# jermp/sshash

Measured on AMD Instinct MI355X. Metric: k-mer Lookups/sec (batched random queries, bit-exact ids), higher is better.
Workload: dtype u64

## Files before the change

sshash_amd/_binding.py:

```python
from __future__ import annotations

import ctypes as C
import os
import sys
from dataclasses import dataclass
from typing import Callable, Iterable, Optional, Sequence, Union

import numpy as np

INVALID_U64 = 0xFFFFFFFFFFFFFFFF

_HERE = os.path.dirname(os.path.abspath(__file__))
_LIB_NAME = "libsshash_amd.so"


def library_path() -> str:
    return os.environ.get("SSHASH_AMD_LIBRARY") or os.path.join(_HERE, _LIB_NAME)


class SSHashError(RuntimeError):

    def __init__(self, status: int, message: str):
        super().__init__(f"[sshash status {status}] {message}")
        self.status = status
# ... 326 lines not shown
    def weighted(self) -> bool: return bool(self._info.weighted)

    def to_device(self, device: int = 0, table_shards: int = 1, table_shard_id: int = 0) -> "Dictionary":
        if table_shards > 1:
            _check(_load().sshash_to_device_table_shard(self._h, int(device), int(table_shards), int(table_shard_id)))
            return self
        _check(_load().sshash_to_device(self._h, int(device)))
        return self

    def device_bytes(self, device: int = 0) -> int:
        out = C.c_uint64()
        _check(_load().sshash_device_bytes(self._h, int(device), C.byref(out)))
        return int(out.value)

    def bucket_stats(self) -> dict:
        out = (C.c_uint64 * 64)()
        _check(_load().sshash_bucket_stats(self._h, C.byref(out)))
        v = [int(x) for x in out]
        return {"num_minimizers": v[0], "num_minimizer_positions": v[1], "num_buckets_larger_than_1_not_in_skew_index": v[2],
                "num_minimizer_positions_of_buckets_larger_than_1": v[3], "num_buckets_in_skew_index": v[4],
                "num_minimizer_positions_of_buckets_in_skew_index": v[5], "num_kmers_in_skew_index": v[6], "max_bucket_size": v[7],
                "num_kmers_in_skew_partition": v[8:8 + v[35]], "buckets_with_n_positions": v[16:32], "num_kmers": v[32],
                "num_strings": v[33], "num_bases": v[34], "max_string_length": v[36]}

    def device_stats(self, device: int = 0) -> dict:
        out = (C.c_uint64 * 16)()
        _check(_load().sshash_device_stats(self._h, int(device), C.byref(out)))
        reasons = {0: None, 1: "disabled", 2: "minimizer shard", 3: "more than 2^39 bases", 4: "too many items for one build pass",
                   5: "not enough free HBM"}
        return {"bytes": int(out[0]), "directory_sectors": int(out[1]), "directory_overflow_sectors": int(out[2]),
                "directory_keys": int(out[3]), "sk_slots": int(out[4]), "sk_keys": int(out[5]), "sk_inline_keys": int(out[6]),
                "sk_deferred_keys": int(out[7]), "sk_slots_used": int(out[8]), "sk_heavy_keys": int(out[9]),
                "sk_heavy_kmers": int(out[10]), "sk_absent_reason": reasons.get(int(out[11]), str(int(out[11]))),
                "sk_bytes": int(out[12]), "sk_key_length": int(out[13]), "sk_load_factor": round(int(out[8]) / int(out[4]), 4) if int(out[4]) else 0.0}

    def device_table_histogram(self, device: int = 0) -> dict:
        out = (C.c_uint64 * 32)()
        _check(_load().sshash_device_table_histogram(self._h, int(device), C.byref(out)))
        v = [int(x) for x in out]
        bins = ["1", "2", "3", "4", "5-8", "9-16", "17-64", "65-1024", ">1024"]
        return {"keys_by_occurrences": dict(zip(bins, v[0:9])), "super_kmers_by_occurrences_of_their_key": dict(zip(bins, v[9:18])),
                "super_kmers": v[18], "slots_asked_for": v[19]}

    def _as_batch(self, kmers: KmerBatch):
        if isinstance(kmers, (str, bytes)):
            kmers = [kmers]
        if isinstance(kmers, np.ndarray) and kmers.dtype == np.uint64:
            a = np.ascontiguousarray(kmers)
            w = self.words_per_kmer()
            if a.size % w:
                raise ValueError("packed k-mer array length is not a multiple of words_per_kmer")
            return False, a, a.size // w
        if isinstance(kmers, np.ndarray) and kmers.dtype == np.uint8:
            a = np.ascontiguousarray(kmers)
            if a.size % self.k():
                raise ValueError("ASCII k-mer buffer length is not a multiple of k")
            return True, a, a.size // self.k()
        a = encode_kmers(list(kmers), self.k())
        return True, np.ascontiguousarray(a), a.shape[0]

    def lookup(self, kmers: KmerBatch, check_reverse_complement: bool = True, full: bool = False,
               out: Optional[np.ndarray] = None) -> LookupResult:
        is_ascii, a, n = self._as_batch(kmers)
        if out is not None and (out.dtype != np.uint64 or out.size != n or not out.flags["C_CONTIGUOUS"]):
            raise ValueError("out must be a contiguous uint64 array with one entry per k-mer")
        res = LookupResult(kmer_id=out if out is not None else np.empty(n, dtype=np.uint64))
        r = _Results()
# ... 393 lines not shown
```

sshash_amd/csrc/engine.hip:

```cpp
#include <hip/hip_runtime.h>

#include <algorithm>
#include <atomic>
#include <cstdlib>
#include <cstring>
#include <mutex>
#include <exception>
#include <stdexcept>
#include <thread>

#include "engine.hpp"
#include "hooks.hpp"
#include "replica.hpp"
#include "sktable.hpp"

namespace sshash_amd {

static void check_single_launch(uint64_t lanes, char const* what) {
    if (lanes >= (uint64_t(1) << 32))
        throw error(error_kind::argument, std::string(what) + ": at most 2^32 - 1 lanes per call (split the batch)");
}


int visible_device_count() {
// ... 124 lines not shown
    std::shared_lock<std::shared_mutex> lock(m_replicas_mutex);
    for (auto const& r : m_replicas)
        if (r->device == device) return true;
    return false;
}

std::vector<int> engine::devices() const {
    std::vector<int> d;
    std::shared_lock<std::shared_mutex> lock(m_replicas_mutex);
    for (auto const& r : m_replicas) d.push_back(r->device);
    return d;
}

uint64_t engine::device_bytes(int device) const { return replica(device)->bytes; }

void engine::device_stats(int device, uint64_t out[16]) const {
    device_replica const* r = replica(device);
    out[0] = r->bytes;
    out[1] = r->view.directory.enabled ? r->view.directory.num_buckets : 0;
    out[2] = r->directory_overflowed;
    out[3] = r->directory_entries;
    out[4] = r->view.sk.enabled ? uint64_t(r->view.sk.num_buckets) * SK_BUCKET_SLOTS +
                                      uint64_t(r->view.sk.kmer_buckets) * (r->view.k > 31 ? SK_BUCKET_SLOTS : SK_KMER_ENTRIES_NARROW)
                                : 0;
    out[5] = r->sk_keys;
    out[6] = r->sk_keys - r->sk_heavy_keys;
    out[7] = r->sk_unplaced;
    out[8] = r->sk_slots_used;
    out[9] = r->sk_heavy_keys;
    out[10] = r->sk_heavy_kmers;
    out[11] = r->view.sk.enabled ? 0 : r->sk_absent_reason;
    out[12] = r->sk_bytes;
    out[13] = r->view.sk.m;
    out[14] = out[15] = 0;
}

void engine::device_table_histogram(int device, uint64_t out[32]) const {
    device_replica const* r = replica(device);
    for (int i = 0; i < 32; ++i) out[i] = i < 20 && r->view.sk.enabled ? r->sk_histogram[i] : 0;
}

device_replica const* engine::replica(int device) const {
    std::shared_lock<std::shared_mutex> lock(m_replicas_mutex);
    for (auto const& r : m_replicas)
        if (r->device == device) return r.get();
    throw error(error_kind::no_device, "dictionary is not resident on device " + std::to_string(device) +
                             " (call sshash_to_device first)");
}

char const* isa_guard_state() {
#if defined(SSHASH_ISA_GUARDED)
    return "guarded";
#else
    return "plain";
#endif
}

void engine::to_device(int device, uint32_t table_shards, uint32_t table_shard_id) {
#if !defined(SSHASH_ISA_GUARDED)
    {
        static std::once_flag once;
        std::call_once(once, [] {
            fprintf(stderr, "[sshash_amd] WARNING: this library was NOT built through tools/isa_guard.py (make -C sshash_amd/csrc): on gfx950 a "
                                "kernel that keeps a 64-bit shift amount in the last VGPR of its allocation computes wrongly some of the time "
                                "(HISTORY.md); tests/test_isa_guard.py names the kernels of a build that are exposed\n");
        });
    }
// ... 32 lines not shown
        std::vector<granule> g = make_granules(idx, nt);
        if (idx.k <= 31) {
            std::vector<atom32> a = make_atoms(g, nt);
            std::vector<granule>().swap(g);
            v.granules = rep->put(a);
        } else {
            v.granules = rep->put(g);
        }
    }
    v.endpoints = rep->put(idx.endpoints);
    v.minimizers = rep->put_mphf(idx.minimizers_mphf);
    v.cw_width = idx.control_codewords.width;
    v.off_width = idx.mid_load_buckets.width;
    v.begin_buckets_of_size = rep->put(idx.begin_buckets_of_size);
    v.mid_load = rep->put(idx.mid_load_buckets.words);
    v.heavy_load = rep->put(idx.heavy_load_buckets.words);
    v.heavy_size = idx.heavy_load_buckets.size;
    v.codewords = nullptr;
    v.cw_packed = 0;
    v.directory.buckets = nullptr;
    v.directory.num_buckets = 0;
    v.directory.enabled = 0;
    rep->bytes_still_to_come = 8 * sizeof(skew_part_dev);
    for (uint32_t p = 0; p < 8; ++p) {
        if (p < idx.skew_num_partitions && idx.skew_mphfs[p].num_keys) {
            mphf_host const& f = idx.skew_mphfs[p];
            rep->bytes_still_to_come += f.parts.size() * sizeof(f.parts[0]) + (f.pilots.size() + f.free_slots.size() + idx.skew_positions[p].words.size()) * 8;
        } else {
            rep->bytes_still_to_come += 64;
        }
    }
    if (idx.weighted()) rep->bytes_still_to_come += (idx.weight_starts.size() + idx.weight_values.size()) * 8;
    build_sk_table(*rep, idx, table_shards, table_shard_id);
    const char* dir_env = std::getenv("SSHASH_AMD_DIRECTORY");
    const bool lean = v.sk.enabled && !(dir_env && dir_env[0] == '1');
    if (lean) {
        v.codewords = rep->put(idx.control_codewords.words);
        v.cw_packed = 1;
    } else {
        const uint64_t n = idx.control_codewords.size;
        device_buffers tmp;
        uint64_t* packed = tmp.alloc<uint64_t>(idx.control_codewords.words.size());
        HIP_CHECK(hipMemcpy(packed, idx.control_codewords.words.data(), idx.control_codewords.words.size() * sizeof(uint64_t), hipMemcpyHostToDevice));
        uint64_t* wide = tmp.alloc<uint64_t>(std::max<uint64_t>(n, 1));
        tmp.keep(wide, *rep);
        rep->bytes += std::max<uint64_t>(n, 1) * sizeof(uint64_t);
        if (n) {
            check_single_launch(n, "upload (one lane per minimizer)");
            hipLaunchKernelGGL(widen_codewords_kernel, dim3(uint32_t((n + 255) / 256)), dim3(256), 0, 0, v, packed, n, wide);
            HIP_CHECK(hipGetLastError());
            HIP_CHECK(hipDeviceSynchronize());
        }
        v.codewords = wide;
    }
    if (!lean) {
        const bool want = !(dir_env && dir_env[0] == '0');
        const uint64_t n = idx.control_codewords.size;
        const uint64_t nb = uint64_t(double(n) / DIR_LOAD) + 1;
        if (want && n && nb < (uint64_t(1) << 32) && v.cw_width <= DIR_CODE_BITS) {
            device_buffers tmp;
            uint64_t* buckets = tmp.alloc<uint64_t>(nb * 4);
            uint32_t* claimed = tmp.alloc<uint32_t>(nb);
            unsigned long long* stats = tmp.alloc<unsigned long long>(2);
            HIP_CHECK(hipMemset(buckets, 0, nb * 32));
            HIP_CHECK(hipMemset(claimed, 0, nb * 4));
            HIP_CHECK(hipMemset(stats, 0, 16));
// ... 76 lines not shown
    }
}

constexpr uint32_t DEFER_SHARDS = 2048;
constexpr uint32_t DEFER_BLOCKS_PER_SHARD = 4;

struct pass_queues {
    uint32_t* defer_counts;
    uint32_t* resume_counts;
    uint32_t* defer_index;
    uint32_t* resume_index;
    uint64_t* resume_kmers;
    uint64_t* resume_meta;
    uint32_t defer_capacity;
    uint32_t resume_capacity;
    uint32_t flag_misses;
};
constexpr uint32_t DEFER_FLAG_ONLY = 1u << 31;

template <int W, bool ASCII>
__device__ __forceinline__ kmer_w<W> load_query(const void* __restrict__ queries, uint64_t i, uint32_t k) {
    kmer_w<W> x;
    if constexpr (ASCII) {
        x = kmer_from_ascii<W>(static_cast<const char*>(queries) + i * k, k);
    } else {
        const uint64_t* q = static_cast<const uint64_t*>(queries) + i * W;
        for (int j = 0; j < W; ++j) x.w[j] = __builtin_nontemporal_load(q + j);
        x = kmer_take_chars<W>(x, k);
    }
    return x;
}

template <int W, bool CANON, int MODE, bool ASCII, bool SK>
__global__ void __launch_bounds__(256, (W == 2 && SK) ? 8 : 1)
fast_lookup_kernel(const dict_view d, const void* __restrict__ queries, const uint64_t n, const bool check_rc,
                   const result_view out, uint8_t* __restrict__ member, const pass_queues q,
                   const uint8_t* __restrict__ lane_valid ) {
    constexpr uint32_t TILE_WORDS = ASCII ? 64 * (W == 1 ? 31 : 63) + 24 : 0;
    constexpr uint32_t STAGE_WORDS = SK ? 256 * 16 : 0;
    __shared__ uint4 lds[(TILE_WORDS > STAGE_WORDS ? TILE_WORDS : STAGE_WORDS) / 4 + 1];
    const uint64_t i = uint64_t(blockIdx.x) * blockDim.x + threadIdx.x;
    const bool active = i < n && (!lane_valid || (lane_valid[i] & 1));
    kmer_w<W> x = kmer_zero<W>();
    if constexpr (ASCII) {
        uint32_t* tile = reinterpret_cast<uint32_t*>(lds);
        const uint64_t first = uint64_t(blockIdx.x) * blockDim.x;
        const uint32_t count = uint32_t(n - first < blockDim.x ? n - first : blockDim.x);
        const uint32_t bytes = count * d.k;
        const char* src = static_cast<const char*>(queries) + first * d.k;
        if ((reinterpret_cast<uintptr_t>(src) & 15) == 0) {
            for (uint32_t c = threadIdx.x; c * 16 < bytes; c += blockDim.x) {
                if (c * 16 + 16 <= bytes) {
                    reinterpret_cast<uint4*>(tile)[c] = sk_load_piece(src + 16 * c);
                } else {
                    for (uint32_t b = c * 16; b < bytes; ++b) reinterpret_cast<char*>(tile)[b] = src[b];
                }
            }
        } else {
            for (uint32_t b = threadIdx.x; b < bytes; b += blockDim.x) reinterpret_cast<char*>(tile)[b] = src[b];
        }
        __syncthreads();
        if (active) {
            const uint32_t start = threadIdx.x * d.k, w0 = start >> 2, sh = start & 3;
            uint32_t acc[2 * W];
#pragma unroll
            for (int t = 0; t < 2 * W; ++t) {
                acc[t] = 0;
                if (16u * uint32_t(t) < d.k) {
                    uint32_t prev = tile[w0 + 4 * t];
#pragma unroll
                    for (int j = 0; j < 4; ++j) {
                        const uint32_t next = tile[w0 + 4 * t + j + 1];
                        const uint32_t four = __builtin_amdgcn_alignbyte(next, prev, sh);
                        prev = next;
                        const uint32_t c = (((four >> 1) & 0x03030303u) * 0x01041040u) >> 24;
                        acc[t] |= c << (8 * j);
                    }
                }
            }
            x.w[0] = uint64_t(acc[0]) | (uint64_t(acc[1]) << 32);
            if constexpr (W == 2) x.w[1] = uint64_t(acc[2]) | (uint64_t(acc[3]) << 32);
            x = kmer_take_chars<W>(x, d.k);
        }
        if constexpr (SK) __syncthreads();
    } else {
        if (active) x = load_query<W, false>(queries, i, d.k);
    }
    fast_t r;
    const uint32_t shard = blockIdx.x & (DEFER_SHARDS - 1);
    if constexpr (SK) {
        if constexpr (W == 1)
            r = sk_lookup_in_wave<W>(d, x, active, CANON || check_rc, (!CANON && check_rc) ? int8_t(-1) : int8_t(1), lds + (threadIdx.x >> 6) * (64 * 4));
        else
            r = sk_first_pass_wave<W>(d, x, active, CANON || check_rc, (!CANON && check_rc) ? int8_t(-1) : int8_t(1),
                                      lds + (threadIdx.x >> 6) * (64 * 4));
        bool resume = active && r.outcome == FAST_CONTINUE;
        const uint32_t place = wave_queue_place(resume, q.resume_counts + shard);
        if (resume) {
            if (place < q.resume_capacity) {
                const uint64_t at = uint64_t(shard) * q.resume_capacity + place;
                q.resume_index[at] = uint32_t(i) | uint32_t(r.kmer_offset);
                for (int j = 0; j < W; ++j) q.resume_kmers[at * W + j] = x.w[j];
            } else {
                r.outcome = FAST_DEFER;
            }
        }
        if (!active) return;
    } else {
        bool by_pairs = false;
        if constexpr (W == 1 && !CANON) by_pairs = (d.num_bases >> 37) == 0;
        if (by_pairs) {
            if constexpr (W == 1 && !CANON) r = fast_lookup_pairs(d, x, active, check_rc);
        } else {
            r = active ? fast_lookup_one<W, CANON>(d, x, check_rc) : fast_unsettled(false);
        }
        const bool scan = active && r.outcome == FAST_SCAN;
        const uint32_t place = wave_queue_place(scan, q.resume_counts + shard);
        if (scan) {
            if (place < q.resume_capacity) {
                const uint64_t at = uint64_t(shard) * q.resume_capacity + place;
                q.resume_index[at] = uint32_t(i);
                q.resume_meta[at] = r.kmer_offset;
                for (int j = 0; j < W; ++j) q.resume_kmers[at * W + j] = x.w[j];
            } else {
                r.outcome = FAST_DEFER;
            }
        }
        if (!active) return;
// ... 1016 lines not shown
                HIP_CHECK(hipMemcpyAsync(dp, hp, m * bytes_per_query, hipMemcpyHostToDevice, s));
            }
            if (ASCII) eng.lookup_ascii_device(device, dp, m, check_rc, mode, d_out, d_member, s);
            else eng.lookup_packed_device(device, reinterpret_cast<uint64_t const*>(dp), m, check_rc, mode, d_out, d_member, s);
            if (in_place) {
                if (member) HIP_CHECK(hipMemcpyAsync(member + at, d_member, m, hipMemcpyDeviceToHost, s));
                for_each_field([&](int, auto* h, auto* d, uint64_t width) {
                    if (h) HIP_CHECK(hipMemcpyAsync(h + at, d, m * width, hipMemcpyDeviceToHost, s));
                }, want, d_out);
                HIP_CHECK(hipStreamSynchronize(s));
                continue;
            }
            HIP_CHECK(hipMemcpyAsync(h_out_block, d_out_block, out_bytes, hipMemcpyDeviceToHost, s));
            HIP_CHECK(hipStreamSynchronize(s));
            if (member) std::memcpy(member + at, h_out_block, m);
            for_each_field([&](int, auto* h, auto* staged_h, uint64_t width) {
                if (h) std::memcpy(h + at, staged_h, m * width);
            }, want, h_stage);
        }
    });
}

void engine::lookup_packed_host(uint64_t const* h_kmers, uint64_t n, bool check_rc, out_mode mode,
                                result_view const& h_out, uint8_t* h_member) const {
    host_lookup<false>(*this, h_kmers, 8ull * m_idx->words_per_kmer(), n, check_rc, mode, h_out, h_member);
}

void engine::lookup_ascii_host(char const* h_kmers, uint64_t n, bool check_rc, out_mode mode, result_view const& h_out,
                               uint8_t* h_member) const {
    host_lookup<true>(*this, h_kmers, m_idx->k, n, check_rc, mode, h_out, h_member);
}

}
```

sshash_amd/csrc/lookup_device.hpp:

```cpp
#pragma once

#include <hip/hip_runtime.h>

#include "device_layout.hpp"

namespace sshash_amd {

struct skew_part_dev {
    mphf_view f;
    uint64_t const* positions;
    uint32_t pos_width;
    uint32_t pad;
};

struct hit_t {
    uint64_t kmer_offset;
    uint32_t string_id;
    int8_t orientation;
    bool found;
    bool minimizer_found;
};

template <int W>
struct window_t {
// ... 529 lines not shown
    if (__ballot(second) != 0) {
        const kmer_w<1> x_rc = kmer_revcomp<1>(x, d.k);
        const minimizer_t mr = compute_minimizer<1>(x_rc, d.k, d.m, d.hash_magic);
        const fast_t r2 = fast_probe_regular_pairs(d, x_rc, mr, true, fast_resolve_pairs(d, mr.value, second), second);
        if (second) {
            r = r2;
            r.orientation = -1;
        }
    }
    return r;
}

template <int W, bool CANON>
__device__ __forceinline__ fast_t fast_lookup_one(dict_view const& d, kmer_w<W> const& x, bool check_rc) {
    if constexpr (CANON) {
        const kmer_w<W> x_rc = kmer_revcomp<W>(x, d.k);
        const minimizer_t mf = compute_minimizer<W>(x, d.k, d.m, d.hash_magic);
        const minimizer_t mr = compute_minimizer<W>(x_rc, d.k, d.m, d.hash_magic);
        if (mf.value == mr.value) return fast_unsettled(true);
        return fast_probe_canonical<W>(d, x, x_rc, mf.value < mr.value ? mf : mr);
    } else {
        const minimizer_t mf = compute_minimizer<W>(x, d.k, d.m, d.hash_magic);
        fast_t r = fast_probe_regular<W>(d, x, mf, false, fast_resolve(d, mf.value));
        if (r.outcome == FAST_MISS && check_rc) {
            const kmer_w<W> x_rc = kmer_revcomp<W>(x, d.k);
            const minimizer_t mr = compute_minimizer<W>(x_rc, d.k, d.m, d.hash_magic);
            r = fast_probe_regular<W>(d, x_rc, mr, true, fast_resolve(d, mr.value));
            r.orientation = -1;
        }
        return r;
    }
}

__device__ __forceinline__ bool sk_usable(dict_view const& d, sk_key_t const& kk) {
    return !kk.tie && (d.sk.num_shards <= 1 || sk_owner(kk.key, d.sk.num_shards) == d.sk.shard_id);
}

template <int W>
struct sk_query_t {
    kmer_w<W> y, y_rc;
    uint32_t j;
    uint32_t fingerprint;
    bool s;
};

template <int W>
__device__ __forceinline__ sk_query_t<W> sk_make_query(kmer_w<W> const& x, kmer_w<W> const& x_rc, sk_key_t const& kk,
                                                        uint32_t fingerprint) {
    sk_query_t<W> q;
    q.s = kk.rc;
    q.j = kk.pos;
    q.y = kk.rc ? x_rc : x;
    q.y_rc = kk.rc ? x : x_rc;
    q.fingerprint = fingerprint;
    return q;
}

template <int W>
__device__ __forceinline__ kmer_w<W> kmer_pick(bool first, kmer_w<W> const& a, kmer_w<W> const& b) {
    kmer_w<W> out;
    for (int t = 0; t < W; ++t) out.w[t] = first ? a.w[t] : b.w[t];
    return out;
}

__device__ __forceinline__ uint32_t sk_choice(sk_hash_t const& h, uint32_t c) {
    return c == 0 ? h.bucket[0] : c == 1 ? h.bucket[1] : c == 2 ? h.bucket[2] : c == 3 ? h.bucket[3] : h.bucket[4];
}

struct sk_bucket_flags {
    uint32_t go_on;
    bool second_used;
};

template <int W, bool FIRST, bool TRACK, class Piece>
__device__ __forceinline__ void sk_examine_slot_tracking(dict_view const& d, sk_query_t<W> const Q, uint32_t c, Piece piece, fast_t& r,
                                                         bool& key_seen, bool& marker, sk_bucket_flags& flags, uint32_t& lasts, bool& inline_seen) {
    const uint32_t km = d.k - d.sk.m;
    const uint32_t j = Q.j;
    kmer_w<W> y, y_rc;
    for (int t = 0; t < W; ++t) {
        y.w[t] = Q.y.w[t];
        y_rc.w[t] = Q.y_rc.w[t];
    }
    const uint4 q0 = piece(0), q1 = piece(1);
    uint4 q2 = q1;
    if constexpr (W == 2) q2 = piece(2);
    const uint32_t meta = q0.x;
    if constexpr (FIRST) {
        uint32_t go_on = meta & (SK_GO_ON << c);
        if (c == 0) go_on &= 0u - ((meta >> (SK_FILTER_SHIFT + sk_filter_index(Q.fingerprint))) & 1u);
        asm volatile("" : "+v"(go_on));
        flags.go_on = go_on;
        flags.second_used = (meta & SK_SECOND_USED) != 0;
        if constexpr (W == 2) {
            const uint4 spare = piece(SK_SECOND_FINGERPRINT_WORD / 4);
            flags.second_used = flags.second_used && spare.x == Q.fingerprint;
        }
    }
    const bool valid = (meta & SK_VALID) != 0, is_marker = (meta & SK_MARKER) != 0;
    const bool same_fingerprint = valid && (q0.w >> 8) == Q.fingerprint;
    key_seen = key_seen || same_fingerprint;
    marker = marker || (same_fingerprint && is_marker);
    const uint64_t at = uint64_t(q0.z) | (uint64_t(q0.w & 0xFFu) << 32);
    const bool o = (meta & SK_STRAND) != 0;
    const uint32_t a = o ? j : km - j;
    const uint64_t w0 = uint64_t(q1.x) | (uint64_t(q1.y) << 32), w1 = uint64_t(q1.z) | (uint64_t(q1.w) << 32);
    kmer_w<W> cand;
    if constexpr (W == 1) {
        cand.w[0] = funnel_shr(w0, w1, 2 * a);
    } else {
        const uint64_t w2 = uint64_t(q2.x) | (uint64_t(q2.y) << 32), w3 = uint64_t(q2.z) | (uint64_t(q2.w) << 32);
        const bool up = 2 * a >= 64;
        const uint32_t sh = (2 * a) & 63u;
        const uint64_t e0 = up ? w1 : w0, e1 = up ? w2 : w1, e2 = up ? w3 : w2;
        cand.w[0] = funnel_shr(e0, e1, sh);
        cand.w[1] = funnel_shr(e1, e2, sh);
    }
    cand = kmer_take_chars<W>(cand, d.k);
    const uint32_t left = (meta >> SK_LEFT_SHIFT) & 63u, right = (meta >> SK_RIGHT_SHIFT) & 63u;
    const kmer_w<W> target = kmer_pick<W>(o, y_rc, y);
    const bool hit = valid && !is_marker && kmer_eq<W>(cand, target) && a + left >= km && a <= right;
    r.kmer_offset = hit ? at + a - km : r.kmer_offset;
    r.string_id = hit ? q0.y : r.string_id;
    r.orientation = hit ? ((o != Q.s) ? int8_t(-1) : int8_t(1)) : r.orientation;
    r.outcome = hit ? int(FAST_HIT) : r.outcome;
    if constexpr (TRACK) {
        uint32_t first, last;
        bool differ;
        if constexpr (W == 1) {
            const uint64_t x0 = cand.w[0] ^ target.w[0];
            differ = x0 != 0;
            first = uint32_t(__builtin_ctzll(x0 | (uint64_t(1) << 63))) >> 1;
            last = (63u - uint32_t(__builtin_clzll(x0 | 1u))) >> 1;
        } else {
            const uint64_t x0 = cand.w[0] ^ target.w[0], x1 = cand.w[1] ^ target.w[1];
            differ = (x0 | x1) != 0;
            first = x0 ? uint32_t(__builtin_ctzll(x0)) >> 1 : 32u + (uint32_t(__builtin_ctzll(x1 | (uint64_t(1) << 63))) >> 1);
            last = x1 ? 32u + ((63u - uint32_t(__builtin_clzll(x1))) >> 1) : (63u - uint32_t(__builtin_clzll(x0 | 1u))) >> 1;
        }
        const bool along = o == Q.s;
        uint32_t mine = along ? last : d.k - 1 - first;
        mine = (differ && !is_marker) ? mine : 0u;
        lasts = (same_fingerprint && mine < lasts) ? mine : lasts;
        inline_seen = inline_seen || (same_fingerprint && !is_marker);
    }
}

template <int W, bool FIRST, class Piece>
__device__ __forceinline__ void sk_examine_slot(dict_view const& d, sk_query_t<W> const Q, uint32_t c, Piece piece, fast_t& r,
                                                bool& key_seen, bool& marker, sk_bucket_flags& flags) {
    uint32_t unused = 0;
    bool unused_too = false;
    sk_examine_slot_tracking<W, FIRST, false>(d, Q, c, piece, r, key_seen, marker, flags, unused, unused_too);
}

template <bool FIRST, class Piece>
__device__ __forceinline__ void sk_examine_kmer_entry(sk_query_t<2> const Q, uint32_t c, Piece piece, fast_t& r, sk_bucket_flags& flags) {
    kmer_w<2> y, y_rc;
    for (int t = 0; t < 2; ++t) {
        y.w[t] = Q.y.w[t];
        y_rc.w[t] = Q.y_rc.w[t];
    }
    const uint4 q0 = piece(0), q1 = piece(1);
    const uint32_t meta = q0.x;
    if constexpr (FIRST) {
        uint32_t go_on = meta & (SK_GO_ON << c);
        if (c == 0) go_on &= 0u - ((meta >> (SK_FILTER_SHIFT + sk_filter_index(Q.fingerprint))) & 1u);
        asm volatile("" : "+v"(go_on));
        flags.go_on = go_on;
        flags.second_used = false;
    }
    kmer_w<2> body;
    body.w[0] = uint64_t(q1.x) | (uint64_t(q1.y) << 32);
    body.w[1] = uint64_t(q1.z) | (uint64_t(q1.w) << 32);
    const bool valid = (meta & SK_VALID) != 0;
    const bool as_y = valid && kmer_eq<2>(body, y), as_rc = valid && kmer_eq<2>(body, y_rc);
    const bool hit = as_y || as_rc;
    r.kmer_offset = hit ? (uint64_t(q0.z) | (uint64_t(q0.w & 0xFFu) << 32)) : r.kmer_offset;
    r.string_id = hit ? q0.y : r.string_id;
    r.orientation = hit ? ((as_rc != Q.s) ? int8_t(-1) : int8_t(1)) : r.orientation;
    r.outcome = hit ? int(FAST_HIT) : r.outcome;
}

template <class Word>
__device__ __forceinline__ void sk_examine_kmer_line(sk_query_t<1> const Q, uint32_t c, Word word, fast_t& r, sk_bucket_flags& flags) {
    const uint64_t y = Q.y.w[0], y_rc = Q.y_rc.w[0];
// ... 97 lines not shown
    char const* slots = static_cast<char const*>(d.sk.slots);
    const uint32_t sub = threadIdx.x & 3u;
    const uint32_t mine = need ? bucket : 0u, my_line = need ? line : 0u;
    const uint32_t b0 = quad_broadcast<0>(mine), b1 = quad_broadcast<1>(mine), b2 = quad_broadcast<2>(mine), b3 = quad_broadcast<3>(mine);
    uint32_t l0 = 0, l1 = 0, l2 = 0, l3 = 0;
    if constexpr (W == 2) {
        l0 = quad_broadcast<0>(my_line);
        l1 = quad_broadcast<1>(my_line);
        l2 = quad_broadcast<2>(my_line);
        l3 = quad_broadcast<3>(my_line);
    }
    uint64_t a0 = uint64_t(b0) * (64 * W) + 64 * l0, a1 = uint64_t(b1) * (64 * W) + 64 * l1, a2 = uint64_t(b2) * (64 * W) + 64 * l2,
             a3 = uint64_t(b3) * (64 * W) + 64 * l3;
    if constexpr (W == 2 && MIXED) {
        const uint32_t mine_region = need && kmer_region ? 1u : 0u;
        const uint64_t base = uint64_t(d.sk.num_buckets) * 128, first = d.sk.num_buckets;
        if (quad_broadcast<0>(mine_region)) a0 = base + uint64_t(b0 - first) * 64;
        if (quad_broadcast<1>(mine_region)) a1 = base + uint64_t(b1 - first) * 64;
        if (quad_broadcast<2>(mine_region)) a2 = base + uint64_t(b2 - first) * 64;
        if (quad_broadcast<3>(mine_region)) a3 = base + uint64_t(b3 - first) * 64;
    }
    const uint32_t lane = threadIdx.x & 63u;
    const uint4 p0 = sk_load_piece(slots + a0 + 16 * sub), p1 = sk_load_piece(slots + a1 + 16 * sub),
                p2 = sk_load_piece(slots + a2 + 16 * sub), p3 = sk_load_piece(slots + a3 + 16 * sub);
    wave_stage[0 * 64 + lane] = p0;
    wave_stage[1 * 64 + lane] = p1;
    wave_stage[2 * 64 + lane] = p2;
    wave_stage[3 * 64 + lane] = p3;
    __builtin_amdgcn_fence(__ATOMIC_RELEASE, "wavefront");
    __builtin_amdgcn_wave_barrier();
    __builtin_amdgcn_fence(__ATOMIC_ACQUIRE, "wavefront");
}

template <int W, bool MIXED = false>
__device__ __forceinline__ void sk_probe_bucket_wave(dict_view const& d, sk_query_t<W> const& Q, uint32_t bucket, uint32_t c, bool need,
                                                     uint4* wave_stage, fast_t& r, bool& key_seen, bool& marker, uint32_t& go_on,
                                                     bool kmer_region = false) {
    const uint32_t lane = threadIdx.x & 63u;
    const uint4* mine = wave_stage + (lane & 3u) * 64 + (lane >> 2) * 4;
    sk_bucket_flags flags;
    flags.go_on = 0;
    flags.second_used = false;
    sk_stage_lines<W, MIXED>(d, bucket, 0u, need, wave_stage, kmer_region);
    bool compact = false;
    if constexpr (MIXED) compact = kmer_region;
    if (need && !compact) {
        sk_examine_slot<W, true>(d, Q, c, [mine](uint32_t i) { return mine[i]; }, r, key_seen, marker, flags);
        if constexpr (W == 1) sk_examine_slot<W, false>(d, Q, c, [mine](uint32_t i) { return mine[2 + i]; }, r, key_seen, marker, flags);
    }
    if constexpr (W == 2 && MIXED) {
        if (need && compact) {
            sk_examine_kmer_entry<true>(Q, c, [mine](uint32_t i) { return mine[i]; }, r, flags);
            sk_examine_kmer_entry<false>(Q, c, [mine](uint32_t i) { return mine[2 + i]; }, r, flags);
        }
    }
    if constexpr (W == 1 && MIXED) {
        if (need && compact) {
            const uint32_t* words = reinterpret_cast<const uint32_t*>(mine);
            sk_examine_kmer_line(Q, c, [words](uint32_t i) { return words[i]; }, r, flags);
        }
    }
    if constexpr (W == 2) {
        bool second = need && r.outcome == FAST_MISS && flags.second_used;
        uint32_t* posted = reinterpret_cast<uint32_t*>(wave_stage + 64);
        char const* slots = static_cast<char const*>(d.sk.slots);
#pragma unroll 1
        for (;;) {
            sk_wave_sync();
            const uint64_t mask = __ballot(second);
            if (mask == 0) break;
            const uint32_t rank = uint32_t(__popcll(mask & ((uint64_t(1) << lane) - 1)));
            const bool served = second && rank < 16;
            if (lane < 16) posted[lane] = 0u;
            sk_wave_sync();
            if (served) posted[rank] = bucket;
            sk_wave_sync();
            const uint32_t b = posted[lane >> 2];
            wave_stage[lane] = sk_load_piece(slots + uint64_t(b) * 128 + 64 + 16 * (lane & 3u));
            sk_wave_sync();
            if (served) {
                const uint4* line = wave_stage + 4 * rank;
                sk_examine_slot<W, false>(d, Q, c, [line](uint32_t i) { return line[i]; }, r, key_seen, marker, flags);
                second = false;
            }
        }
    }
    go_on = flags.go_on;
    __builtin_amdgcn_wave_barrier();
}

constexpr uint32_t RESUME_CHOICE_SHIFT = 27;
constexpr uint32_t RESUME_HEAVY = 1u << 30;
constexpr uint32_t RESUME_GO_ON = 1u << 31;

template <int W>
__device__ __forceinline__ fast_t sk_first_pass_wave(dict_view const& d, kmer_w<W> const& x, bool active, bool allow_rc,
                                                     int8_t miss_orientation, uint4* wave_stage) {
    const kmer_w<W> x_rc = kmer_revcomp<W>(x, d.k);
    const sk_key_t kk = sk_key<W>(x, x_rc, d.k, d.sk.m);
    const bool usable = active && sk_usable(d, kk);
    const sk_hash_t h = sk_hash(kk.key, d.sk.num_buckets);
    const sk_query_t<W> Q = sk_make_query<W>(x, x_rc, kk, h.fingerprint);
    fast_t r = fast_unsettled(active && !usable);
    uint32_t go_on = 0;
    bool marker = false, key_seen = false;
    sk_probe_bucket_wave<W>(d, Q, usable ? h.bucket[0] : 0u, 0u, usable, wave_stage, r, key_seen, marker, go_on);
    if constexpr (W == 2) {
        bool hop = usable && r.outcome == FAST_MISS && marker;
        if (__ballot(hop) != 0) {
            const sk_hash_t hk = sk_hash_kmer_region(sk_kmer_key<W>(x, x_rc), d.sk.num_buckets, d.sk.kmer_buckets);
            sk_query_t<W> Qk = Q;
            Qk.fingerprint = hk.fingerprint;
            const uint32_t lane = threadIdx.x & 63u;
            uint32_t* posted = reinterpret_cast<uint32_t*>(wave_stage + 64);
            char const* slots = static_cast<char const*>(d.sk.slots);
            uint32_t kmer_go_on = 0;
            bool pending = hop;
#pragma unroll 1
            for (;;) {
                sk_wave_sync();
                const uint64_t mask = __ballot(pending);
                if (mask == 0) break;
                const uint32_t rank = uint32_t(__popcll(mask & ((uint64_t(1) << lane) - 1)));
                const bool served = pending && rank < 16;
                if (lane < 16) posted[lane] = 0u;
                sk_wave_sync();
                if (served) posted[rank] = 2 * d.sk.num_buckets + (hk.bucket[0] - d.sk.num_buckets);
                sk_wave_sync();
                const uint32_t line = posted[lane >> 2];
                wave_stage[lane] = sk_load_piece(slots + uint64_t(line) * 64 + 16 * (lane & 3u));
                sk_wave_sync();
                if (served) {
                    const uint4* mine = wave_stage + 4 * rank;
                    sk_bucket_flags flags;
                    sk_examine_kmer_entry<true>(Qk, 0u, [mine](uint32_t i) { return mine[i]; }, r, flags);
                    sk_examine_kmer_entry<false>(Qk, 0u, [mine](uint32_t i) { return mine[2 + i]; }, r, flags);
                    kmer_go_on = flags.go_on;
                    pending = false;
                }
            }
            if (hop && r.outcome == FAST_MISS && kmer_go_on == 0) {
                marker = false;
            }
        }
    }
    if (usable) {
        if (r.outcome == FAST_MISS) {
            if (marker) {
                r.outcome = FAST_CONTINUE;
                r.kmer_offset = RESUME_HEAVY | (go_on ? RESUME_GO_ON : 0u);
            } else if (go_on) {
                r.outcome = FAST_CONTINUE;
                r.kmer_offset = 1u << RESUME_CHOICE_SHIFT;
            } else {
                r.orientation = miss_orientation;
            }
        } else if (r.orientation < 0 && !allow_rc) {
            r = fast_unsettled(false);
            r.orientation = miss_orientation;
        }
    }
    return r;
}

__device__ __forceinline__ void sk_finish_in_wave(dict_view const& d, kmer_w<1> const& x, kmer_w<1> const& x_rc, sk_key_t const& kk, sk_walk_t& w,
                                                  sk_query_t<1>& Q, fast_t& r, bool need, uint4* wave_stage) {
    const uint32_t lane = threadIdx.x & 63u;
    char const* slots = static_cast<char const*>(d.sk.slots);
    uint32_t* posted = reinterpret_cast<uint32_t*>(wave_stage + 64);
#pragma unroll 1
    for (;;) {
        const uint64_t mask = __ballot(need);
        if (mask == 0) break;
        const uint32_t rank = uint32_t(__popcll(mask & ((uint64_t(1) << lane) - 1)));
        const bool served = need && rank < 16;
        if (lane < 16) posted[lane] = 0u;
        sk_wave_sync();
        if (served) posted[rank] = sk_choice(w.h, w.c);
        sk_wave_sync();
        const uint32_t b = posted[lane >> 2];
        wave_stage[lane] = sk_load_piece(slots + uint64_t(b) * 64 + 16 * (lane & 3u));
        sk_wave_sync();
        if (served) {
            const uint4* mine = wave_stage + 4 * rank;
            sk_bucket_flags flags;
            flags.go_on = 0;
            flags.second_used = false;
            bool marker = false, key_seen = false;
            if (sk_choice(w.h, w.c) >= d.sk.num_buckets) {
                const uint32_t* words = reinterpret_cast<const uint32_t*>(mine);
                sk_examine_kmer_line(Q, w.c, [words](uint32_t i) { return words[i]; }, r, flags);
            } else {
                sk_examine_slot<1, true>(d, Q, w.c, [mine](uint32_t i) { return mine[i]; }, r, key_seen, marker, flags);
                sk_examine_slot<1, false>(d, Q, w.c, [mine](uint32_t i) { return mine[2 + i]; }, r, key_seen, marker, flags);
// ... 20 lines not shown
    sk_wave_sync();
    bool need = false;
    if (usable) need = sk_walk_step<W>(d, x, x_rc, kk, w, Q, r, go_on, marker);
    sk_finish_in_wave(d, x, x_rc, kk, w, Q, r, need, wave_stage);
    if (usable && (r.outcome == FAST_MISS || (r.outcome == FAST_HIT && r.orientation < 0 && !allow_rc))) {
        r = fast_unsettled(false);
        r.orientation = miss_orientation;
    }
    return r;
}

template <int W>
__device__ __forceinline__ fast_t sk_second_pass_wave(dict_view const& d, kmer_w<W> const& x, bool active, uint32_t entry, bool allow_rc,
                                                      int8_t miss_orientation, uint4* wave_stage) {
    const kmer_w<W> x_rc = kmer_revcomp<W>(x, d.k);
    const sk_key_t kk = sk_key<W>(x, x_rc, d.k, d.sk.m);
    sk_walk_t w = sk_walk_begin(sk_hash(kk.key, d.sk.num_buckets), (entry >> RESUME_CHOICE_SHIFT) & 7u);
    sk_query_t<W> Q = sk_make_query<W>(x, x_rc, kk, w.h.fingerprint);
    if (entry & RESUME_HEAVY) sk_walk_to_kmer_sequence<W>(d, x, x_rc, w, Q, (entry & RESUME_GO_ON) != 0);
    fast_t r = fast_unsettled(false);
    bool need = active;
#pragma unroll 1
    while (__ballot(need) != 0) {
        uint32_t go_on = 0;
        bool marker = false, key_seen = false;
        const uint32_t bucket = need ? sk_choice(w.h, w.c) : 0u;
        sk_probe_bucket_wave<W, true>(d, Q, bucket, w.c, need, wave_stage, r, key_seen, marker, go_on, bucket >= d.sk.num_buckets);
        if (need) need = sk_walk_step<W>(d, x, x_rc, kk, w, Q, r, go_on, marker);
    }
    if (r.outcome == FAST_MISS || (r.outcome == FAST_HIT && r.orientation < 0 && !allow_rc)) {
        r = fast_unsettled(false);
        r.orientation = miss_orientation;
    }
    return r;
}

__device__ __forceinline__ uint32_t wave_queue_place(bool push, uint32_t* counter) {
    const uint64_t mask = __ballot(push);
    if (mask == 0) return 0;
    const uint32_t lane = threadIdx.x & 63u;
    const uint32_t leader = uint32_t(__ffsll((unsigned long long)mask)) - 1u;
    uint32_t base = 0;
    if (lane == leader) base = atomicAdd(counter, uint32_t(__popcll(mask)));
    base = __shfl(base, int(leader), 64);
    return base + uint32_t(__popcll(mask & ((uint64_t(1) << lane) - 1)));
}

template <bool FULL>
__device__ __forceinline__ void store_result(dict_view const& d, result_view const& out, uint64_t i, hit_t const& h) {
    __builtin_nontemporal_store(h.found ? h.kmer_offset - uint64_t(h.string_id) * (d.k - 1) : INVALID_U64, out.kmer_id + i);
    if constexpr (FULL) {
        uint64_t begin = INVALID_U64, end = INVALID_U64;
        if (h.found && (out.string_begin || out.string_end || out.kmer_id_in_string)) {
            begin = d.endpoints[h.string_id];
            end = d.endpoints[h.string_id + 1];
        }
        if (out.kmer_id_in_string) __builtin_nontemporal_store(h.found ? h.kmer_offset - begin : INVALID_U64, out.kmer_id_in_string + i);
        if (out.kmer_offset) __builtin_nontemporal_store(h.found ? h.kmer_offset : INVALID_U64, out.kmer_offset + i);
        if (out.string_id) __builtin_nontemporal_store(h.found ? uint64_t(h.string_id) : INVALID_U64, out.string_id + i);
        if (out.string_begin) __builtin_nontemporal_store(begin, out.string_begin + i);
        if (out.string_end) __builtin_nontemporal_store(end, out.string_end + i);
        if (out.kmer_orientation) __builtin_nontemporal_store(h.orientation, out.kmer_orientation + i);
        if (out.minimizer_found) __builtin_nontemporal_store(uint8_t(h.minimizer_found ? 1 : 0), out.minimizer_found + i);
    }
}

// ... 2 lines not shown
```

sshash_amd/csrc/replica.hpp:

```cpp
#pragma once

#include <algorithm>
#include <atomic>

#include <cstdio>
#include <cstdlib>

#include <hip/hip_runtime.h>

#include <functional>
#include <mutex>
#include <stdexcept>
#include <string>
#include <unordered_map>
#include <vector>

#include "lookup_device.hpp"
#include "mphf_build.hpp"

namespace sshash_amd {

inline void hip_check(hipError_t e, char const* what) {
    if (e != hipSuccess) throw error(error_kind::hip, std::string("HIP error in ") + what + ": " + hipGetErrorString(e));
}
// ... 61 lines not shown
    void release(void* stream) {
        std::lock_guard<std::mutex> lock(m_mutex);
        auto it = m_slots.find(stream);
        if (it == m_slots.end()) return;
        it->second.slot.release();
        m_slots.erase(it);
    }
    void clear() {
        std::lock_guard<std::mutex> lock(m_mutex);
        for (auto& kv : m_slots) kv.second.slot.release();
        m_slots.clear();
    }

private:
    struct entry {
        Slot slot;
        uint64_t last_use = 0;
    };
    std::mutex m_mutex;
    std::unordered_map<void*, entry> m_slots;
    uint64_t m_clock = 0;
};

struct device_replica {
    int device = -1;
    uint64_t bytes = 0;
    uint64_t bytes_still_to_come = 0;
    dict_view view{};
    skew_part_dev* d_skew = nullptr;
    uint64_t directory_overflowed = 0;
    uint64_t directory_entries = 0;
    uint64_t sk_keys = 0, sk_heavy_keys = 0, sk_heavy_kmers = 0, sk_unplaced = 0, sk_slots_used = 0, sk_bytes = 0;
    uint32_t sk_absent_reason = 1;
    uint64_t sk_histogram[20] = {0};
    std::vector<void*> allocations;
    hipMemPool_t scratch_pool = nullptr;
    void create_scratch_pool() {
        hipMemPoolProps props{};
        props.allocType = hipMemAllocationTypePinned;
        props.handleTypes = hipMemHandleTypeNone;
        props.location.type = hipMemLocationTypeDevice;
        props.location.id = device;
        if (hipMemPoolCreate(&scratch_pool, &props) != hipSuccess) {
            scratch_pool = nullptr;
            (void)hipGetLastError();
            if (std::getenv("SSHASH_AMD_VERBOSE"))
                fprintf(stderr, "[sshash_amd] device %d: no private memory pool (hipMemPoolCreate failed): stream-ordered scratch comes out of the default pool\n", device);
            return;
        }
        uint64_t keep = ~uint64_t(0);
        (void)hipMemPoolSetAttribute(scratch_pool, hipMemPoolAttrReleaseThreshold, &keep);
    }
    void* stream_alloc(size_t bytes, hipStream_t s) const {
        void* p = nullptr;
        if (scratch_pool) HIP_CHECK(hipMallocFromPoolAsync(&p, bytes ? bytes : 8, scratch_pool, s));
        else HIP_CHECK(hipMallocAsync(&p, bytes ? bytes : 8, s));
        return p;
    }

    mutable std::mutex launch_mutex;
    struct stream_scratch : stream_block {
        hipStream_t aux = nullptr;
        hipEvent_t first_done[2] = {nullptr, nullptr};
        hipEvent_t tail_done[2] = {nullptr, nullptr};
        void free_block() {
            if (aux) HIP_CHECK(hipStreamSynchronize(aux));
// ... 147 lines not shown
```

Before: 39.43 billion.

## Stage whole super-k-mer buckets per octet for wide k-mers and lower occupancy hint

For W==2 non-mixed probes, each group of eight lanes now loads the first 96 bytes of all eight lanes' buckets, using ds_swizzle broadcasts to share bucket indices, and stages them into a padded LDS layout. Each lane then examines both slots from LDS in one pass instead of the older line-by-line staging, and skips the separate second-fingerprint check. The LDS stage buffer grows and the launch-bounds wave hint drops from 8 to 6 to leave room for more registers. The change also adds a build-time bucket census exposed through device_stats, plus compile-gated probe counters.

```diff
diff --git a/sshash_amd/_binding.py b/sshash_amd/_binding.py
--- a/sshash_amd/_binding.py
+++ b/sshash_amd/_binding.py
@@ -382,7 +382,8 @@
                 "directory_keys": int(out[3]), "sk_slots": int(out[4]), "sk_keys": int(out[5]), "sk_inline_keys": int(out[6]),
                 "sk_deferred_keys": int(out[7]), "sk_slots_used": int(out[8]), "sk_heavy_keys": int(out[9]),
                 "sk_heavy_kmers": int(out[10]), "sk_absent_reason": reasons.get(int(out[11]), str(int(out[11]))),
-                "sk_bytes": int(out[12]), "sk_key_length": int(out[13]), "sk_load_factor": round(int(out[8]) / int(out[4]), 4) if int(out[4]) else 0.0}
+                "sk_bytes": int(out[12]), "sk_key_length": int(out[13]),
+                "sk_second_slot_buckets": int(out[14]), "sk_go_on_buckets": int(out[15]), "sk_load_factor": round(int(out[8]) / int(out[4]), 4) if int(out[4]) else 0.0}
 
     def device_table_histogram(self, device: int = 0) -> dict:
         out = (C.c_uint64 * 32)()
diff --git a/sshash_amd/csrc/engine.hip b/sshash_amd/csrc/engine.hip
--- a/sshash_amd/csrc/engine.hip
+++ b/sshash_amd/csrc/engine.hip
@@ -180,7 +180,37 @@
     out[11] = r->view.sk.enabled ? 0 : r->sk_absent_reason;
     out[12] = r->sk_bytes;
     out[13] = r->view.sk.m;
-    out[14] = out[15] = 0;
+    out[14] = r->sk_second_slot_buckets;
+    out[15] = r->sk_go_on_buckets;
+}
+
+__global__ void __launch_bounds__(256)
+sk_census_kernel(const uint32_t* __restrict__ slots, const uint64_t num_buckets, const uint32_t words_per_bucket, unsigned long long* __restrict__ out) {
+    const uint64_t stride = uint64_t(gridDim.x) * blockDim.x;
+    uint32_t second = 0, go_on = 0;
+    for (uint64_t b = uint64_t(blockIdx.x) * blockDim.x + threadIdx.x; b < num_buckets; b += stride) {
+        const uint32_t meta = slots[b * words_per_bucket];
+        second += (meta & SK_SECOND_USED) != 0;
+        go_on += (meta & (((1u << SK_CHOICES) - 1u) * SK_GO_ON)) != 0;
+    }
+    if (second) atomicAdd(out, (unsigned long long)second);
+    if (go_on) atomicAdd(out + 1, (unsigned long long)go_on);
+}
+
+static void sk_census(device_replica& rep) {
+    sk_view const& sk = rep.view.sk;
+    if (!sk.enabled || sk.num_buckets == 0) return;
+    device_buffers tmp;
+    unsigned long long* counts = tmp.alloc<unsigned long long>(2);
+    HIP_CHECK(hipMemset(counts, 0, 2 * sizeof(unsigned long long)));
+    const uint32_t words_per_bucket = rep.view.k <= 31 ? 16u : 32u;
+    const uint32_t blocks = uint32_t(std::min<uint64_t>((uint64_t(sk.num_buckets) + 255) / 256, 4096));
+    sk_census_kernel<<<blocks, 256>>>(static_cast<const uint32_t*>(sk.slots), sk.num_buckets, words_per_bucket, counts);
+    HIP_CHECK(hipGetLastError());
+    unsigned long long h[2] = {0, 0};
+    HIP_CHECK(hipMemcpy(h, counts, sizeof h, hipMemcpyDeviceToHost));
+    rep.sk_second_slot_buckets = h[0];
+    rep.sk_go_on_buckets = h[1];
 }
 
 void engine::device_table_histogram(int device, uint64_t out[32]) const {
@@ -279,6 +309,7 @@
     }
     if (idx.weighted()) rep->bytes_still_to_come += (idx.weight_starts.size() + idx.weight_values.size()) * 8;
     build_sk_table(*rep, idx, table_shards, table_shard_id);
+    sk_census(*rep);
     const char* dir_env = std::getenv("SSHASH_AMD_DIRECTORY");
     const bool lean = v.sk.enabled && !(dir_env && dir_env[0] == '1');
     if (lean) {
@@ -421,12 +452,13 @@
 }
 
 template <int W, bool CANON, int MODE, bool ASCII, bool SK>
-__global__ void __launch_bounds__(256, (W == 2 && SK) ? 8 : 1)
+__global__ void __launch_bounds__(256, (W == 2 && SK) ? 6 : 1)
 fast_lookup_kernel(const dict_view d, const void* __restrict__ queries, const uint64_t n, const bool check_rc,
                    const result_view out, uint8_t* __restrict__ member, const pass_queues q,
                    const uint8_t* __restrict__ lane_valid ) {
     constexpr uint32_t TILE_WORDS = ASCII ? 64 * (W == 1 ? 31 : 63) + 24 : 0;
-    constexpr uint32_t STAGE_WORDS = SK ? 256 * 16 : 0;
+    constexpr uint32_t STAGE_PIECES = W == 2 ? SK_WHOLE_STAGE_PIECES : 64 * 4;
+    constexpr uint32_t STAGE_WORDS = SK ? 4 * STAGE_PIECES * 4 : 0;
     __shared__ uint4 lds[(TILE_WORDS > STAGE_WORDS ? TILE_WORDS : STAGE_WORDS) / 4 + 1];
     const uint64_t i = uint64_t(blockIdx.x) * blockDim.x + threadIdx.x;
     const bool active = i < n && (!lane_valid || (lane_valid[i] & 1));
@@ -479,10 +511,10 @@
     const uint32_t shard = blockIdx.x & (DEFER_SHARDS - 1);
     if constexpr (SK) {
         if constexpr (W == 1)
-            r = sk_lookup_in_wave<W>(d, x, active, CANON || check_rc, (!CANON && check_rc) ? int8_t(-1) : int8_t(1), lds + (threadIdx.x >> 6) * (64 * 4));
+            r = sk_lookup_in_wave<W>(d, x, active, CANON || check_rc, (!CANON && check_rc) ? int8_t(-1) : int8_t(1), lds + (threadIdx.x >> 6) * STAGE_PIECES);
         else
             r = sk_first_pass_wave<W>(d, x, active, CANON || check_rc, (!CANON && check_rc) ? int8_t(-1) : int8_t(1),
-                                      lds + (threadIdx.x >> 6) * (64 * 4));
+                                      lds + (threadIdx.x >> 6) * STAGE_PIECES);
         bool resume = active && r.outcome == FAST_CONTINUE;
         const uint32_t place = wave_queue_place(resume, q.resume_counts + shard);
         if (resume) {
@@ -1565,3 +1597,17 @@
 }
 
 }
+
+#ifdef SSHASH_SK_STATS
+extern "C" int sshash_debug_sk_stats(uint64_t* out, int count, int clear) {
+    unsigned long long v[sshash_amd::SK_STAT_COUNT] = {};
+    hipError_t e = hipDeviceSynchronize();
+    if (e == hipSuccess) e = hipMemcpyFromSymbol(v, HIP_SYMBOL(sshash_amd::sk_stat_counters), sizeof v);
+    for (int i = 0; i < count; ++i) out[i] = i < int(sshash_amd::SK_STAT_COUNT) ? v[i] : 0;
+    if (e == hipSuccess && clear) {
+        const unsigned long long zero[sshash_amd::SK_STAT_COUNT] = {};
+        e = hipMemcpyToSymbol(HIP_SYMBOL(sshash_amd::sk_stat_counters), zero, sizeof zero);
+    }
+    return int(e);
+}
+#endif
diff --git a/sshash_amd/csrc/lookup_device.hpp b/sshash_amd/csrc/lookup_device.hpp
--- a/sshash_amd/csrc/lookup_device.hpp
+++ b/sshash_amd/csrc/lookup_device.hpp
@@ -585,6 +585,36 @@
     }
 }
 
+enum sk_stat : int {
+    SK_STAT_ACTIVE = 0,
+    SK_STAT_PROBES,
+    SK_STAT_SLOT0_HITS,
+    SK_STAT_SLOT1_IN_USE,
+    SK_STAT_SLOT1_WANTED,
+    SK_STAT_SLOT1_HITS,
+    SK_STAT_HOPS,
+    SK_STAT_HOP_HITS,
+    SK_STAT_RESUME_HEAVY,
+    SK_STAT_RESUME_GO_ON,
+    SK_STAT_DEFERRED,
+    SK_STAT_WAVES,
+    SK_STAT_RANKED_TURNS,
+    SK_STAT_RESUME_BUCKETS,
+    SK_STAT_RESUME_DEFERRED,
+    SK_STAT_COUNT
+};
+#ifdef SSHASH_SK_STATS
+static __device__ unsigned long long sk_stat_counters[SK_STAT_COUNT];
+#define SK_STAT(which, pred)                                                                                        \
+    do {                                                                                                            \
+        const unsigned long long sk_stat_all = __ballot(true), sk_stat_set = __ballot(pred);                        \
+        if (sk_stat_set && (threadIdx.x & 63u) == uint32_t(__ffsll(sk_stat_all)) - 1u)                              \
+            atomicAdd(&sk_stat_counters[which], (unsigned long long)__popcll(sk_stat_set));                         \
+    } while (0)
+#else
+#define SK_STAT(which, pred) (void)0
+#endif
+
 __device__ __forceinline__ bool sk_usable(dict_view const& d, sk_key_t const& kk) {
     return !kk.tie && (d.sk.num_shards <= 1 || sk_owner(kk.key, d.sk.num_shards) == d.sk.shard_id);
 }
@@ -625,7 +655,7 @@
     bool second_used;
 };
 
-template <int W, bool FIRST, bool TRACK, class Piece>
+template <int W, bool FIRST, bool TRACK, bool WHOLE = false, class Piece>
 __device__ __forceinline__ void sk_examine_slot_tracking(dict_view const& d, sk_query_t<W> const Q, uint32_t c, Piece piece, fast_t& r,
                                                          bool& key_seen, bool& marker, sk_bucket_flags& flags, uint32_t& lasts, bool& inline_seen) {
     const uint32_t km = d.k - d.sk.m;
@@ -645,7 +675,7 @@
         asm volatile("" : "+v"(go_on));
         flags.go_on = go_on;
         flags.second_used = (meta & SK_SECOND_USED) != 0;
-        if constexpr (W == 2) {
+        if constexpr (W == 2 && !WHOLE) {
             const uint4 spare = piece(SK_SECOND_FINGERPRINT_WORD / 4);
             flags.second_used = flags.second_used && spare.x == Q.fingerprint;
         }
@@ -699,12 +729,12 @@
     }
 }
 
-template <int W, bool FIRST, class Piece>
+template <int W, bool FIRST, bool WHOLE = false, class Piece>
 __device__ __forceinline__ void sk_examine_slot(dict_view const& d, sk_query_t<W> const Q, uint32_t c, Piece piece, fast_t& r,
                                                 bool& key_seen, bool& marker, sk_bucket_flags& flags) {
     uint32_t unused = 0;
     bool unused_too = false;
-    sk_examine_slot_tracking<W, FIRST, false>(d, Q, c, piece, r, key_seen, marker, flags, unused, unused_too);
+    sk_examine_slot_tracking<W, FIRST, false, WHOLE>(d, Q, c, piece, r, key_seen, marker, flags, unused, unused_too);
 }
 
 template <bool FIRST, class Piece>
@@ -868,15 +898,71 @@
     __builtin_amdgcn_fence(__ATOMIC_ACQUIRE, "wavefront");
 }
 
+constexpr uint32_t SK_WHOLE_STAGE_PIECES = 416;
+
+template <int OWNER>
+__device__ __forceinline__ uint32_t octet_broadcast(uint32_t v) {
+    return uint32_t(__builtin_amdgcn_ds_swizzle(int(v), 0x18 | (OWNER << 5)));
+}
+
+__device__ __forceinline__ uint32_t sk_whole_place(uint32_t owner ) { return 6 * owner + 7 * (((owner >> 3) & 1u) + (owner >> 4)); }
+
+__device__ __forceinline__ void sk_stage_buckets_whole(dict_view const& d, uint32_t bucket, bool need, uint4* wave_stage) {
+    char const* slots = static_cast<char const*>(d.sk.slots);
+    const uint32_t lane = threadIdx.x & 63u, sub = lane & 7u;
+    const uint32_t mine = need ? bucket : 0u;
+    const uint32_t b0 = octet_broadcast<0>(mine), b1 = octet_broadcast<1>(mine), b2 = octet_broadcast<2>(mine), b3 = octet_broadcast<3>(mine),
+                   b4 = octet_broadcast<4>(mine), b5 = octet_broadcast<5>(mine), b6 = octet_broadcast<6>(mine), b7 = octet_broadcast<7>(mine);
+    if ((sub & 3u) != 3u) {
+        char const* from = slots + 16 * sub;
+        const uint4 p0 = sk_load_piece(from + uint64_t(b0) * 128), p1 = sk_load_piece(from + uint64_t(b1) * 128),
+                    p2 = sk_load_piece(from + uint64_t(b2) * 128), p3 = sk_load_piece(from + uint64_t(b3) * 128),
+                    p4 = sk_load_piece(from + uint64_t(b4) * 128), p5 = sk_load_piece(from + uint64_t(b5) * 128),
+                    p6 = sk_load_piece(from + uint64_t(b6) * 128), p7 = sk_load_piece(from + uint64_t(b7) * 128);
+        uint4* to = wave_stage + sk_whole_place(lane & 56u) + (sub - (sub >> 2));
+        to[0] = p0;
+        to[6] = p1;
+        to[12] = p2;
+        to[18] = p3;
+        to[24] = p4;
+        to[30] = p5;
+        to[36] = p6;
+        to[42] = p7;
+    }
+    __builtin_amdgcn_fence(__ATOMIC_RELEASE, "wavefront");
+    __builtin_amdgcn_wave_barrier();
+    __builtin_amdgcn_fence(__ATOMIC_ACQUIRE, "wavefront");
+}
+
 template <int W, bool MIXED = false>
 __device__ __forceinline__ void sk_probe_bucket_wave(dict_view const& d, sk_query_t<W> const& Q, uint32_t bucket, uint32_t c, bool need,
                                                      uint4* wave_stage, fast_t& r, bool& key_seen, bool& marker, uint32_t& go_on,
                                                      bool kmer_region = false) {
     const uint32_t lane = threadIdx.x & 63u;
-    const uint4* mine = wave_stage + (lane & 3u) * 64 + (lane >> 2) * 4;
     sk_bucket_flags flags;
     flags.go_on = 0;
     flags.second_used = false;
+    if constexpr (W == 2 && !MIXED) {
+        sk_stage_buckets_whole(d, bucket, need, wave_stage);
+        const uint4* mine = wave_stage + sk_whole_place(lane);
+        if (need) {
+            sk_examine_slot<W, true, true>(d, Q, c, [mine](uint32_t i) { return mine[i]; }, r, key_seen, marker, flags);
+#ifdef SSHASH_SK_STATS
+            const bool open = r.outcome == FAST_MISS;
+            SK_STAT(SK_STAT_SLOT0_HITS, !open);
+            SK_STAT(SK_STAT_SLOT1_IN_USE, open && (mine[0].x & SK_SECOND_USED) != 0);
+            SK_STAT(SK_STAT_SLOT1_WANTED, open && (mine[3].x & SK_VALID) != 0 && (mine[3].w >> 8) == Q.fingerprint);
+#endif
+            sk_examine_slot<W, false, true>(d, Q, c, [mine](uint32_t i) { return mine[3 + i]; }, r, key_seen, marker, flags);
+#ifdef SSHASH_SK_STATS
+            SK_STAT(SK_STAT_SLOT1_HITS, open && r.outcome == FAST_HIT);
+#endif
+        }
+        go_on = flags.go_on;
+        sk_wave_sync();
+        return;
+    }
+    const uint4* mine = wave_stage + (lane & 3u) * 64 + (lane >> 2) * 4;
     sk_stage_lines<W, MIXED>(d, bucket, 0u, need, wave_stage, kmer_region);
     bool compact = false;
     if constexpr (MIXED) compact = kmer_region;
@@ -921,6 +1007,7 @@
             }
         }
     }
+    if constexpr (MIXED) SK_STAT(SK_STAT_RESUME_BUCKETS, need);
     go_on = flags.go_on;
     __builtin_amdgcn_wave_barrier();
 }
@@ -941,8 +1028,12 @@
     uint32_t go_on = 0;
     bool marker = false, key_seen = false;
     sk_probe_bucket_wave<W>(d, Q, usable ? h.bucket[0] : 0u, 0u, usable, wave_stage, r, key_seen, marker, go_on);
+    SK_STAT(SK_STAT_WAVES, (threadIdx.x & 63u) == 0);
+    SK_STAT(SK_STAT_ACTIVE, active);
+    SK_STAT(SK_STAT_PROBES, usable);
     if constexpr (W == 2) {
         bool hop = usable && r.outcome == FAST_MISS && marker;
+        SK_STAT(SK_STAT_HOPS, hop);
         if (__ballot(hop) != 0) {
             const sk_hash_t hk = sk_hash_kmer_region(sk_kmer_key<W>(x, x_rc), d.sk.num_buckets, d.sk.kmer_buckets);
             sk_query_t<W> Qk = Q;
@@ -957,6 +1048,7 @@
                 sk_wave_sync();
                 const uint64_t mask = __ballot(pending);
                 if (mask == 0) break;
+                SK_STAT(SK_STAT_RANKED_TURNS, lane == 0);
                 const uint32_t rank = uint32_t(__popcll(mask & ((uint64_t(1) << lane) - 1)));
                 const bool served = pending && rank < 16;
                 if (lane < 16) posted[lane] = 0u;
@@ -975,6 +1067,7 @@
                     pending = false;
                 }
             }
+            SK_STAT(SK_STAT_HOP_HITS, hop && r.outcome == FAST_HIT);
             if (hop && r.outcome == FAST_MISS && kmer_go_on == 0) {
                 marker = false;
             }
@@ -996,6 +1089,9 @@
             r.orientation = miss_orientation;
         }
     }
+    SK_STAT(SK_STAT_RESUME_HEAVY, r.outcome == FAST_CONTINUE && (uint32_t(r.kmer_offset) & RESUME_HEAVY) != 0);
+    SK_STAT(SK_STAT_RESUME_GO_ON, r.outcome == FAST_CONTINUE && (uint32_t(r.kmer_offset) & RESUME_HEAVY) == 0);
+    SK_STAT(SK_STAT_DEFERRED, r.outcome == FAST_DEFER);
     return r;
 }
 
@@ -1082,6 +1178,7 @@
         r = fast_unsettled(false);
         r.orientation = miss_orientation;
     }
+    SK_STAT(SK_STAT_RESUME_DEFERRED, active && r.outcome == FAST_DEFER);
     return r;
 }
 
diff --git a/sshash_amd/csrc/replica.hpp b/sshash_amd/csrc/replica.hpp
--- a/sshash_amd/csrc/replica.hpp
+++ b/sshash_amd/csrc/replica.hpp
@@ -117,6 +117,7 @@
     uint64_t directory_entries = 0;
     uint64_t sk_keys = 0, sk_heavy_keys = 0, sk_heavy_kmers = 0, sk_unplaced = 0, sk_slots_used = 0, sk_bytes = 0;
     uint32_t sk_absent_reason = 1;
+    uint64_t sk_second_slot_buckets = 0, sk_go_on_buckets = 0;
     uint64_t sk_histogram[20] = {0};
     std::vector<void*> allocations;
     hipMemPool_t scratch_pool = nullptr;
```

Result: no change. 39.37 billion, median of 2 (-0.2%).
